# edsonportosilva/OptiCommPy

Measured on AMD Instinct MI355X. Metric: SSFM steps/sec (2-pol, 2^20 samples), higher is better.
Workload: dtype f64

## Files before the change

opticommpy_amd/csrc/engine_fused_impl.h:

```cpp
#pragma once
#include <algorithm>
#include <cstdlib>
#include <vector>

#include "dev_ctx.h"
#include "fused_engine.h"
#include "ssf_internal.h"

namespace ssf {
namespace {

using namespace fused;

#ifdef SSF_PHASE_TIMING
__device__ unsigned long long g_marks[4][4096][8];
#endif

struct DevCtx : DevCtxCore {
#ifdef SSF_PHASE_TIMING
    int kind;
    unsigned long long ts[8] = {0, 0, 0, 0, 0, 0, 0, 0};
    __device__ __forceinline__ void mark(int i) {
        __builtin_amdgcn_sched_barrier(0);
#if SSF_PHASE_TIMING != 2
// ... 244 lines not shown
        if (lg1 == 8 && cols == 8) return pick_col_sg_d<T, 8>(sg);
        if (lg1 == 9 && cols == 8) return pick_col_sg_d<T, 9>(sg);
    } else if constexpr (std::is_same<T, pf2>::value) {
        if (lg1 == 10 && cols == 4) return pick_col_sg_pk<10>(sg);
        if (lg1 == 9 && cols == 8) return pick_col_sg_pk<9>(sg);
    }
    return nullptr;
}
template <typename T> ColFn<T> pick_col(int lg1, int mode) {
    switch (lg1) {
    case 7: return pick_col_mode<T, 7>(mode);
    case 8: return pick_col_mode<T, 8>(mode);
    case 9: return pick_col_mode<T, 9>(mode);
    default: return pick_col_mode<T, 0>(mode);
    }
}

struct HipBackend {
    ssf_plan *pl;
    hipError_t first_err = hipSuccess;
    std::string where;
    hipEvent_t ev0 = nullptr, ev1 = nullptr;

    int row_occ = 2;
    bool col_il = false;
    bool profiling = false;
    struct Stamp { hipEvent_t a, b; int cat; };
    std::vector<Stamp> stamps;
    std::vector<hipEvent_t> pool;
    ssf_kernel_times kt{};
    hipEvent_t get_event() {
        if (!pool.empty()) { hipEvent_t e = pool.back(); pool.pop_back(); return e; }
        hipEvent_t e = nullptr;
        chk(hipEventCreate(&e), "hipEventCreate");
        return e;
    }
    void stamp_begin(int cat) {
        if (!profiling) return;
        Stamp s{get_event(), get_event(), cat};
        chk(hipEventRecord(s.a, pl->stream), "hipEventRecord");
        stamps.push_back(s);
    }
    void stamp_end() {
        if (!profiling) return;
        chk(hipEventRecord(stamps.back().b, pl->stream), "hipEventRecord");
    }
// ... 544 lines not shown
```

opticommpy_amd/csrc/fused_engine.h:

```cpp
#pragma once
#include <algorithm>
#include <cmath>
#include <cstdlib>
#include <cstring>
#include <memory>
#include <string>
#include <type_traits>
#include <vector>

#include "fused_kernels.h"
#include "ssf_derived.h"

namespace ssf {
namespace fused {

#ifndef SSF_EXPERIMENTS
#define SSF_EXPERIMENTS 0
#endif
static inline const char *tune_env(const char *name) {
#if SSF_EXPERIMENTS
    return std::getenv(name);
#else
    (void)name;
    return nullptr;
// ... 111 lines not shown
        }
    }
    return best < 1e300;
}

static inline bool choose_nonpow2_split(int64_t N, int precision, int f1, int fc, bool l1_forced, int *l1, int *N1, int *N2, int *C) {
    *l1 = *N1 = *N2 = *C = 0;
    if (f1 > 0 && choose_mixed2_split(N, precision, N1, N2, C, f1, fc)) return true;
    if (!choose_mixed_split(N, precision, l1, N2)) {
        *l1 = *N2 = 0;
        return choose_mixed2_split(N, precision, N1, N2, C);
    }
    if (*l1 < 7 && !l1_forced) {
        int n1 = 0, n2 = 0, c = 0;
        if (choose_mixed2_split(N, precision, &n1, &n2, &c)) {
            *l1 = 0;
            *N1 = n1;
            *N2 = n2;
            *C = c;
        }
    }
    return true;
}

template <typename T, class Backend> class FusedCore {
  public:
    using C = cx<T>;
    using S = scalar_t<T>;
    static constexpr bool kPacked = sizeof(T) != sizeof(S);
    Backend &be;
    int64_t N;
    int nrows, log2N;
    Split sp;
    int N2mix = 0;
    int mix_rows = 1;
    MixPlan mix_plan{};
    cx<double> *wtab = nullptr;
    int N1mix = 0, mix_cols = 0;
    MixPlan mix_plan1{};
    cx<double> *wtab1 = nullptr;
    int n1() const { return N1mix ? N1mix : 1 << sp.l1; }
    int row_tw_off = 0;
    size_t field_bytes;
    C *G = nullptr, *T0 = nullptr, *T1 = nullptr, *Ehd = nullptr, *noise_d = nullptr;
    S *P = nullptr, *Theta = nullptr;
    bool own_G = true;
    void *cpl_comm = nullptr;
    double *cpl_work = nullptr;
    std::unique_ptr<FusedCore<pf2, Backend>> pk;
    bool use_packed = true;
    bool lim0_bound = true;
    Ctrl *ctrl = nullptr;
    LinOp *linops = nullptr;
    unsigned *gbar = nullptr;
    double *part = nullptr;
    double *tr_hz = nullptr, *tr_lim = nullptr;
    int *tr_it = nullptr;
    long long tr_cap = 0;
    int tr_maxIter = 0;
    std::vector<C *> snaps;
    int row_v = 16;
    int col_v = 16;
    bool underfilled = false;
    int lanes_hint = 1;
    int col_split = 1;
    bool split_ok = true;
    int split_penalty = 0;
    static constexpr int kSplitPenalty = 8;
    int hint_n_it = 0;
    int cur = 0;
    unsigned seq = 0;
    int row_block, row_grid, col_block_mk, col_grid_mk, col_block_1, col_grid_1, npart_max;
    size_t row_lds, col_lds_mk, col_lds_1;
    std::string err;

    std::vector<ssf_stats> ustats;
    int units = 1;
    int npairs() const { return kPacked ? nrows : std::max(nrows / 2, 1); }
    int rows_u() const { return nrows / units; }
    int pairs_u() const { return std::max(npairs() / units, 1); }
    FusedCore(Backend &b, int64_t N_, int nrows_, int precision, void *borrowed_G = nullptr, int units_ = 1)
        : be(b), N(N_), nrows(nrows_), units(units_ > 0 ? units_ : 1) {
        if (borrowed_G) {
            G = (C *)borrowed_G;
            own_G = false;
        }
        log2N = 0;
        while ((1ll << log2N) < N) ++log2N;
        if ((N & (N - 1)) == 0) {
            choose_split(log2N, precision, &sp, kPacked);
        } else {
// ... 16 lines not shown
            *lds = mix2_col_lds(N1mix, mix_cols, npol, (int)sizeof(C));
            return;
        }
        const int tpf = (1 << sp.l1) / col_v, N2 = N2mix ? N2mix : 1 << sp.l2;
        int half = col_v == 8 ? 512 / npol : 256;
        if (const char *e = tune_env("SSF_COL_HALF")) {
            const int h = std::atoi(e);
            if (h >= tpf && h <= 512 && (h & (h - 1)) == 0) half = h;
        }
        while (half / tpf > N2 && half > tpf) half >>= 1;
        auto wgs = [&](int h) { return (long long)groups * (N2 / (h / tpf)); };
        while (!tune_env("SSF_COL_HALF") && half > 64 &&
               ((wgs(half) < 512 && (half / tpf) * sizeof(C) > 128) || (wgs(half) < 256 && (half / tpf) * sizeof(C) > 64)))
            half >>= 1;
        const int Cc = half / tpf;
        *block = half * npol;
        *grid = groups * ((N2 + Cc - 1) / Cc);
        *lds = std::max((size_t)npol * Cc * lds_col_stride(1 << sp.l1, Cc, (int)sizeof(C)) * sizeof(C), (size_t)half * npol * 16 + 1024);
    }

    int init() {
        if (const char *e = tune_env("SSF_LIM0_BOUND")) lim0_bound = std::atoi(e) != 0;
        if (const char *e = tune_env("SSF_COL_SPLIT")) col_split = std::atoi(e);
        underfilled = (double)rows_u() * (double)N <= 1048576.0;
        col_v = underfilled && sp.l1 != 7 ? 8 : 16;
        if (const char *e = tune_env("SSF_COL_V")) col_v = std::atoi(e) == 8 ? 8 : 16;
        if (N2mix || sp.l1 < 6 || sp.l1 > 10) col_v = 16;
        if (N1mix && !mix_make_plan(N1mix, &mix_plan1, 256 / (2 * mix_cols), false)) {
            err = "fused engine: no pass plan for the column length";
            return SSF_ERR_UNSUPPORTED;
        }
        if (const char *e = N1mix ? tune_env("SSF_MIX_PLAN1") : nullptr) {
            int r[kMixMaxPass], n = 0;
            for (const char *q = e; *q && n < kMixMaxPass;) {
                r[n++] = std::atoi(q);
                while (*q && *q != ',') ++q;
                if (*q == ',') ++q;
            }
            MixPlan mp;
            if (mix_plan_from_radices(N1mix, r, n, &mp)) mix_plan1 = mp;
        }
        const int64_t nfft = (int64_t)rows_u() * n1();
        if (N2mix) {
            int tpr = 128;
            if (const char *e = tune_env("SSF_MIX_TPR")) tpr = std::max(64, std::min(1024, std::atoi(e)));
            while (16 * tpr < N2mix) tpr *= 2;
// ... 344 lines not shown

    MkConst mk_const(const ssf_params &p, const Derived &d) const {
        MkConst k{};
        k.Lspan = p.Lspan;
        k.hz_fixed = p.hz;
        k.tol = p.tol;
        k.maxRot = p.maxNlinPhaseRot;
        k.c8g = d.c8g;
        k.sgn = p.direction >= 0 ? 1.0 : -1.0;
        k.lin_a = d.lin_a;
        k.lin_b = d.lin_b;
        k.w2 = (d.w_scale / (double)N) * (d.w_scale / (double)N);
        k.invN = 1.0 / (double)N;
        k.maxIter = p.maxIter;
        k.adaptive = p.nlprMethod ? 1 : 0;
        k.exact_lim0 = (p.maxIter == 1 || !lim0_bound) ? 1 : 0;
        k.log2N = log2N;
        k.trace_cap = tr_cap;
        k.tr_hz = tr_hz;
        k.tr_it = tr_it;
        k.tr_lim = tr_lim;
        return k;
    }
    void launch_mk_row(const MkConst &k) {
        RowArgs<T> a = row_args();
        a.use_ctrl = 1;
        a.cin = ctrl + (size_t)(seq & 1) * units;
        a.cout = ctrl + (size_t)((seq + 1) & 1) * units;
        a.k = k;
        const size_t ps = (size_t)units * (size_t)npart_max;
        a.pmax = part;
        a.pnum = part + ps;
        a.pden = part + 2 * ps;
        a.pnum0 = part + 3 * ps;
        a.pden0 = part + 4 * ps;
        a.npart = col_grid_mk;
        if constexpr (Backend::kCanCouple) {
            if (cpl_comm) {
                if (be.couple(cpl_comm, part, ps, col_grid_mk, cpl_work)) return;
                a.pnum0 = cpl_work;
                a.pden0 = cpl_work + 1;
                a.pnum = cpl_work + 2;
                a.pden = cpl_work + 3;
                a.pmax = cpl_work + 4;
                a.npart = 1;
            }
        }
        be.launch_row(a, row_grid, row_block, row_lds, units);
        ++seq;
// ... 77 lines not shown
                unsigned flags[8] = {0, 0, 0, 0, 0, 0, 0, 0};
                be.d2h(flags, gbar, sizeof(flags));
                if (!be.ok()) return hiperr();
                if (flags[2]) {
                    err = "persistent Manakov kernel: grid barrier timed out (workgroups not co-resident / not on one XCD?)";
                    return SSF_ERR_STATE;
                }
                seq = (seq & ~1u) | (flags[4] & 1u);
                be.d2h(cs.data(), ctrl + (seq & 1), sizeof(Ctrl));
                if (!be.ok()) return hiperr();
                if (cs[0].state != ST_SPAN_DONE || cs[0].pend0) {
                    err = "persistent Manakov kernel: span not finished";
                    return SSF_ERR_STATE;
                }
                persisted = true;
            }
        }
        if (!persisted) {
        launch_mk_col(k, CM_MK);
        int guard = 0;
        long long prev_steps = 0, prev_iters = 0, prev_rare = 0;
        const bool can_split = col_split && split_penalty == 0 && units == 1 && !cpl_comm &&
                               be.can_split_cols(col_args(kPacked ? 1 : 2, CM_MK), col_block_mk);
        bool general_chunk = false;
        int stalls = 0, pos = 0;
        long long idle_pairs = 0;
        for (;;) {
            double steps_rem = 0.0;
            for (const Ctrl &c : cs) {
                double r;
                if (c.state == ST_SPAN_DONE && !c.pend0) r = 0.0;
                else if (c.steps == 0 && c.state == ST_NEED_S) r = p.nlprMethod ? 8.0 : std::ceil(p.Lspan / p.hz);
                else r = std::max(1.0, std::ceil((p.Lspan - c.z) / (c.hz > 0 ? c.hz : p.hz)));
                steps_rem = std::max(steps_rem, r);
            }
            const bool use_split = can_split && split_ok && !general_chunk;
            const int n_pred = std::max(1, std::min(p.maxIter, sr.n_it > 0 ? sr.n_it : (int)std::lround(sr.avg_it)));
            double est = p.nlprMethod ? steps_rem * (1.0 + sr.avg_it) * 0.6
                                      : steps_rem * (1.0 + (use_split ? std::max((double)n_pred, sr.avg_it) : sr.avg_it)) + 3.0;
            int chunk = (int)std::min(512.0, std::max(2.0, std::ceil(est)));
            if (can_split && split_ok && general_chunk) chunk = std::min(chunk, 8);
            else if (use_split && sr.n_it == 0) chunk = std::min(chunk, 4 * (n_pred + 1));
            for (int i = 0; i < chunk; ++i) {
                launch_mk_row(k);
                int sg = SG_ALL;
                if (use_split) {
                    sg = pos == 0 ? (SG_H | SG_RARE) : pos < n_pred ? SG_ADV : SG_FIN;
                    pos = pos >= n_pred ? 0 : pos + 1;
                }
                launch_mk_col(k, CM_MK, sg);
            }
            be.d2h(cs.data(), ctrl + (size_t)(seq & 1) * units, cbytes);
            if (!be.ok()) return hiperr();
            long long steps = 0, iters = 0, rare = 0;
            bool done = true;
            double worst = 0.0;
            for (const Ctrl &c : cs) {
                steps += c.steps;
                iters += c.iterations;
                rare += c.n_rebuilt + c.n_recovered;
                done = done && c.state == ST_SPAN_DONE && !c.pend0;
                if (c.steps > 0) worst = std::max(worst, (double)c.iterations / (double)c.steps);
            }
            if (steps > prev_steps) {
                sr.avg_it = units == 1 ? (double)(iters - prev_iters) / (double)(steps - prev_steps) : worst;
                sr.n_it = cs[0].last_nit;
            }
            if (can_split && split_ok && !done) {
                idle_pairs = steps == prev_steps ? idle_pairs + chunk : 0;
                const bool stuck = idle_pairs >= 2 * (n_pred + 1) + 2;
                if (general_chunk && !stuck) general_chunk = false;
                else if (stuck) {
                    general_chunk = true;
                    if (++stalls >= 2) split_ok = false;
                }
                if (rare - prev_rare > (steps - prev_steps) / 4 + 2) split_ok = false;
                if (!split_ok) split_penalty = kSplitPenalty;
            }
            prev_steps = steps;
            prev_iters = iters;
            prev_rare = rare;
            if (done) break;
            if (++guard > (1 << 22)) {
                err = "fused engine: span did not terminate";
                return SSF_ERR_STATE;
            }
        }
        }
        if (units == 1) {
            cur = cs[0].cur;
        } else {
            const size_t ub = sizeof(C) * (size_t)rows_u() * (size_t)N;
            for (int u = 0; u < units; ++u)
                if (cs[(size_t)u].cur != cur)
// ... 162 lines not shown
```

opticommpy_amd/csrc/fused_kernels.h:

```cpp
#pragma once
#include "fused_core.h"
#include "mixed_fft.h"
#include "ssf_rng.h"

namespace ssf {
namespace fused {

enum {
    ST_NEED_S = 0,
    ST_AFTER_S = 1,
    ST_NEED_H = 2,
    ST_ROW_ITER = 3,
    ST_NEED_I = 4,
    ST_SPAN_DONE = 6,
    ST_REDO0 = 7,
    ST_RECOVER_A = 8,
    ST_RECOVER_ROW = 9,
    ST_RECOVER_B = 10
};

struct LinOp {
    double cth;
    double mag;
    double Cre[9], Cim[9];
};

struct Ctrl {
    int state, it, cur, hz_valid;
    int final_;
    int pend0, pendn;
    int cap0;
    int pcur, redo_;
    int bound0;
    int exact0;
    int t_sparse;
    int dense;
    int gscale;
    int last_nit;
    long long pend0_idx;
    double z, hz;
    long long steps, iterations, nonconv, trace_n;
    long long n_ahead, n_rebuilt;
    long long n_recovered;
    LinOp lin;
};

struct MkConst {
    double Lspan, hz_fixed, tol, maxRot, c8g, sgn, lin_a, lin_b, w2, invN;
    int maxIter, adaptive, log2N;
    int exact_lim0;
    long long trace_cap;
    double *tr_hz;
    int *tr_it;
    double *tr_lim;
};

SSF_HD LinOp make_linop(double hzh, double lin_a, double lin_b, double w2, double invN, int log2N) {
    LinOp l;
    l.cth = lin_b * w2 * hzh;
    l.mag = exp(lin_a * hzh) * invN;
    const double d = (double)(1ll << (log2N - 4));
    for (int m = 0; m < 9; ++m) {
        double s, c;
        cis_rad_d(l.cth * d * d * (double)(m * m), c, s);
        l.Cre[m] = c;
        l.Cim[m] = s;
    }
    return l;
}

SSF_HD double pick_hz(const MkConst &k, double z, double maxphi) {
    if (k.adaptive) {
        const double cand = k.maxRot / maxphi;
        return (k.Lspan - z >= cand) ? cand : k.Lspan - z;
    }
    return (k.Lspan - z < k.hz_fixed) ? k.Lspan - z : k.hz_fixed;
}

SSF_HD cx<double> tw_base(int sign, int j, int lgL) {
    double c, s;
    cis2pi_d(scale_pow2((double)(sign * j), lgL), c, s);
    return mk<double>(c, s);
}
template <int R> SSF_HD void tw_powers(cx<double> w1, cx<double> *p) {
    p[0] = mk<double>(1.0, 0.0);
    p[1] = w1;
    if (R > 2) {
        p[2] = w1 * w1;
        p[3] = p[2] * w1;
    }
    if (R > 4) {
        p[4] = p[2] * p[2];
        p[5] = p[4] * w1;
        p[6] = p[3] * p[3];
        p[7] = p[4] * p[3];
    }
    if (R > 8) {
        p[8] = p[4] * p[4];
#pragma unroll
        for (int s2 = 9; s2 < 16; ++s2) p[s2 < R ? s2 : 0] = p[8] * p[s2 - 8];
// ... 267 lines not shown
    const LinOp *lin;
    const Ctrl *cin;
    Ctrl *cout;
    MkConst k;
    const double *pmax;
    const double *pnum, *pden;
    const double *pnum0, *pden0;
    int npart;
    int N2;
    long long N;
    int mixed;
    MixPlan plan;
    const cx<double> *wtab;
    int rows_per_wg;
    const cx<T> *harr;
    int fwd_only;
    const cx<T> *src;
    int vpt;
    long long u_elems;
    int u_part;
    int prio;
    int tw_off;
    int N1mix;
};
template <typename T> SSF_HD long long row_n1(const RowArgs<T> &a) { return a.N1mix ? (long long)a.N1mix : 1ll << a.log2N1; }

struct Lin16Bases {
    cx<double> A, B1;
    double cth;
};
template <int V = 16> SSF_HD Lin16Bases lin16_bases(double cth, long long k0, int log2N) {
    constexpr int lgV = V == 16 ? 4 : 3;
    const double dk = (double)(1ll << (log2N - lgV));
    const double k0d = (double)k0;
    double s, c;
    Lin16Bases r;
    cis_rad_d(cth * k0d * k0d, c, s);
    r.A = mk<double>(c, s);
    cis_rad_d(2.0 * cth * k0d * dk, c, s);
    r.B1 = mk<double>(c, s);
    r.cth = cth;
    return r;
}
template <int V = 16, typename T> SSF_HD void apply_lin16(const LinOp &lo, const Lin16Bases &lb, cx<T> *v);
template <int V = 16, typename T>
SSF_HD void apply_lin16(const LinOp &lo, long long k0, int log2N, cx<T> *v) {
// ... 40 lines not shown
#if SSF_CTRL_WIDE
    constexpr int kMax = (int)(sizeof(Ctrl) / 8);
    unsigned long long w[kMax];
#pragma unroll
    for (int q = 0; q < kMax; ++q)
        if (q < nwords) w[q] = src[q];
#pragma unroll
    for (int q = 0; q < kMax; ++q)
        if (q < nwords) dst[q] = w[q];
#else
    int i = 0;
    for (; i + 8 <= nwords; i += 8) {
        unsigned long long w[8];
#pragma unroll
        for (int q = 0; q < 8; ++q) w[q] = src[i + q];
#pragma unroll
        for (int q = 0; q < 8; ++q) dst[i + q] = w[q];
    }
    for (; i < nwords; ++i) dst[i] = src[i];
#endif
}

template <typename T, class Ctx>
SSF_HD bool row_ctrl(Ctx &ctx, const RowArgs<T> &a, const double (&part)[2][4], LinOp &lo) {
    LinOp *lsh = (LinOp *)ctx.lds;
    const Ctrl &c = *a.cin;
    const int c_state = c.state, c_it = c.it, c_pend0 = c.pend0, c_pendn = c.pendn, c_cap0 = c.cap0, c_bound0 = c.bound0;
    int n_exact0 = c.exact0;
    const int c_gscale = c.gscale, c_sparse = c.t_sparse;
    int n_state = c_state, n_final = c.final_, n_cap0 = c_cap0, n_hzv = c.hz_valid;
    int add_nonconv = 0, add_ahead = 0;
    const long long c_nonconv = c.nonconv, c_ahead = c.n_ahead;
    double n_hz = c.hz;
    double *red = (double *)(ctx.lds) + 64;
    const bool lead = ctx.bid == 0 && ctx.tid == 0;
    bool act = c_state == ST_AFTER_S || c_state == ST_ROW_ITER || c_state == ST_RECOVER_ROW;
    if (c_pend0 || c_pendn) {
        double s0 = part[0][0] + part[1][0], s1 = part[0][1] + part[1][1];
        double s2 = part[0][2] + part[1][2], s3 = part[0][3] + part[1][3];
        for (int i = ctx.tid + 2 * ctx.nthreads; i < a.npart; i += ctx.nthreads) {
            s0 += a.pnum0[i];
            s1 += a.pden0[i];
            s2 += a.pnum[i];
            s3 += a.pden[i];
        }
        if (c_pend0) block_sum2(ctx, s0, s1, red);
        if (c_pendn) block_sum2(ctx, s2, s3, red);
// ... 37 lines not shown
        ctx.sync();
        if (ctx.tid == 0) {
            const double hz = pick_hz(a.k, c.z, mx);
            lsh[0] = make_linop(hz / 2, a.k.lin_a, a.k.lin_b, a.k.w2, a.k.invN, a.k.log2N);
            ((double *)(lsh + 1))[0] = hz;
        }
        ctx.sync();
        n_hz = ((double *)(lsh + 1))[0];
        lo = lsh[0];
        if (lead) a.cout->lin = lsh[0];
        n_hzv = 1;
        ctx.sync();
    } else if (act && c_state == ST_RECOVER_ROW) {
        ctx.sync();
        if (ctx.tid == 0) lsh[0] = make_linop(-c.hz / 2, a.k.lin_a, a.k.lin_b, a.k.w2, a.k.invN, a.k.log2N);
        ctx.sync();
        lo = lsh[0];
        ctx.sync();
    } else if (act) {
        lo = c.lin;
    }
    if (act && c_state == ST_AFTER_S && c_gscale) lo.mag *= (double)row_n1(a);
    if (act) n_state = c_state == ST_AFTER_S ? ST_NEED_H : c_state == ST_RECOVER_ROW ? ST_RECOVER_B : ST_NEED_I;
    if (lead) {
        ctrl_forward(a.cin, a.cout, (int)((new_lin ? offsetof(Ctrl, lin) : sizeof(Ctrl)) / 8));
        Ctrl *n = a.cout;
        n->state = n_state;
        n->final_ = n_final;
        n->pend0 = 0;
        n->pendn = 0;
        n->cap0 = n_cap0;
        n->bound0 = 0;
        n->exact0 = n_exact0;
        if (n_exact0) n->dense = 1;
        if (act && c_state == ST_AFTER_S) n->gscale = 0;
        n->hz_valid = n_hzv;
        n->hz = n_hz;
        n->nonconv = c_nonconv + add_nonconv;
        n->n_ahead = c_ahead + add_ahead;
    }
    return act;
}

template <typename T> SSF_HD cx<T> lin_at_n(const LinOp &lo, long long k, long long N) {
    const double kk = (double)(k < (N + 1) / 2 ? k : k - N);
    double s, c;
    cis_rad_d(lo.cth * kk * kk, c, s);
    return mk<T>((T)(lo.mag * c), (T)(lo.mag * s));
}

template <typename T, class Ctx> SSF_HD void row_mixed_body(Ctx &ctx, const RowArgs<T> &a, const MixPlan &p) {
    const int L = a.N2, R_ = a.rows_per_wg, T_ = ctx.nthreads / R_;
    const int f = ctx.tid / T_, t = ctx.tid - f * T_;
    cx<T> *x = (cx<T> *)(ctx.lds + 4096) + (size_t)f * L;
    const long long rr = (long long)ctx.bid * R_ + f;
    cx<T> *g = a.G + rr * L;
    const cx<T> *gin = a.src ? a.src + rr * L : g;
    LinOp lo;
// ... 1 lines not shown
#if SSF_EARLY_BASES
    const double cth_pre = a.use_ctrl ? a.cin->lin.cth : (a.lin ? a.lin->cth : 0.0);
#endif
    if (a.use_ctrl) {
#pragma unroll
        for (int u = 0; u < 2; ++u) {
            const int i = ctx.tid + u * ctx.nthreads;
            if (i < a.npart) {
                part[u][0] = a.pnum0[i];
                part[u][1] = a.pden0[i];
                part[u][2] = a.pnum[i];
                part[u][3] = a.pden[i];
            }
        }
        ctx.issue_fence();
    }
    ctx.mark(0);
    const int N1 = (int)row_n1(a);
    const int k1 = a.N1mix ? (int)(rr % N1) : (int)(rr & (N1 - 1));
    MixRowOp op;
    auto ctrl = [&]() {
        if (a.use_ctrl) {
            ctx.issue_fence();
            if (!row_ctrl(ctx, a, part, lo)) return false;
        } else {
            lo = *a.lin;
        }
        const int Rl = p.r[p.npass - 1];
        op.cth = lo.cth;
        op.mag = lo.mag;
        op.D = (double)(a.N / Rl);
        double c, s;
        cis_rad_d(2.0 * lo.cth * op.D * op.D, c, s);
        op.c2 = mk<double>(c, s);
        op.k1 = k1;
        op.N1 = N1;
        op.N = a.N;
        return true;
    };
    if (!mix_dif_op_dit(ctx, p, t, T_, x, a.wtab, op, gin, g, ctrl)) return;
    ctx.mark(4);
    ctx.mark(5);
    ctx.flush(0);
}

#ifndef SSF_WT_ROWS
#define SSF_WT_ROWS 3
#endif
#ifndef SSF_LOAD_ORDER
#define SSF_LOAD_ORDER 1
#endif
#ifndef SSF_EARLY_BASES
#define SSF_EARLY_BASES 0
#endif
#ifndef SSF_SPEC_G
#define SSF_SPEC_G 0
#endif
#ifndef SSF_PAIR_DPP
#define SSF_PAIR_DPP 0
#endif
#ifndef SSF_THETA_F32
#define SSF_THETA_F32 0
#endif
template <typename T> constexpr bool wt_rows() {
    return sizeof(scalar_t<T>) == 8 ? (SSF_WT_ROWS & 1) != 0 : sizeof(T) == 8 ? (SSF_WT_ROWS & 2) != 0 : (SSF_WT_ROWS & 4) != 0;
}
template <int V, typename T, class Ctx>
SSF_HD void row_store(Ctx &ctx, const RowArgs<T> &a, const PassPlan &p, int f, int b, const cx<T> *v) {
    const int fpw = ctx.nthreads / p.tpf;
    cx<T> *base = a.G + (((long long)ctx.bid * fpw) << a.log2N2);
#if defined(__HIP_DEVICE_COMPILE__)
    if constexpr (wt_rows<T>()) {
        const unsigned bytes = (unsigned)(((size_t)fpw << a.log2N2) * sizeof(cx<T>));
        const __amdgpu_buffer_rsrc_t rs = __builtin_amdgcn_make_buffer_rsrc((void *)base, 0, bytes, 0x00020000);
        constexpr int kWT = 0x11;
#pragma unroll
        for (int q = 0; q < V; ++q) {
            const unsigned off = (unsigned)(((f << a.log2N2) + b + p.tpf * q) * (int)sizeof(cx<T>));
            if constexpr (sizeof(cx<T>) == 16) {
                typedef unsigned u4 __attribute__((ext_vector_type(4)));
                u4 w;
                __builtin_memcpy(&w, &v[q], 16);
                __builtin_amdgcn_raw_buffer_store_b128(w, rs, off, 0, kWT);
            } else {
                typedef unsigned u2 __attribute__((ext_vector_type(2)));
                u2 w;
                __builtin_memcpy(&w, &v[q], 8);
                __builtin_amdgcn_raw_buffer_store_b64(w, rs, off, 0, kWT);
            }
        }
        return;
    }
#endif
    cx<T> *g = base + ((long long)f << a.log2N2);
#pragma unroll
    for (int q = 0; q < V; ++q) g[b + p.tpf * q] = v[q];
}

template <typename T, int LG, int V = 16, class Ctx> SSF_HD void row_body(Ctx &ctx, const RowArgs<T> &a) {
    constexpr int lgV = V == 16 ? 4 : 3;
    cx<T> *lds = (cx<T> *)ctx.lds;
    LinOp lo;
    const PassPlan p = make_plan(LG > 0 ? LG : a.log2N2, lgV);
    const int fpw = ctx.nthreads / p.tpf;
    const int f = ctx.tid / p.tpf, b = ctx.tid % p.tpf;
    const long long rr = (long long)ctx.bid * fpw + f;
    cx<T> *g = a.G + (rr << a.log2N2);
    cx<T> v[V];
    ctx.mark(0);
    double part[2][4] = {{0, 0, 0, 0}, {0, 0, 0, 0}};
#if SSF_EARLY_BASES
    const double cth_pre = a.use_ctrl ? a.cin->lin.cth : (a.lin ? a.lin->cth : 0.0);
#endif
    if (a.use_ctrl) {
#pragma unroll
        for (int u = 0; u < 2; ++u) {
            const int i = ctx.tid + u * ctx.nthreads;
            if (i < a.npart) {
                part[u][0] = a.pnum0[i];
                part[u][1] = a.pden0[i];
                part[u][2] = a.pnum[i];
                part[u][3] = a.pden[i];
            }
        }
        ctx.issue_fence();
    }
#if SSF_LOAD_ORDER
    {
        constexpr int ord16[16] = {0, 8, 4, 12, 2, 10, 6, 14, 1, 9, 5, 13, 3, 11, 7, 15};
        constexpr int ord8[8] = {0, 4, 2, 6, 1, 5, 3, 7};
#pragma unroll
        for (int i = 0; i < V; ++i) {
            const int q = V == 16 ? ord16[i] : ord8[i & 7];
            v[q] = g[b + p.tpf * q];
            if ((i & 3) == 3) ctx.issue_fence();
        }
    }
#else
#pragma unroll
    for (int q = 0; q < V; ++q) v[q] = g[b + p.tpf * q];
#endif
    constexpr bool kTab = (SSF_TW_TAB & 1) && sizeof(scalar_t<T>) == 4;
    TwSrc<T> tws;
    if (kTab) {
        tw_entry_t<T> *tab = (tw_entry_t<T> *)(ctx.lds + a.tw_off);
        tw_lds_build<T>(ctx, p, tab);
        tws.lds = tab;
    }
    if (a.use_ctrl) {
        ctx.issue_fence();
        if (!row_ctrl(ctx, a, part, lo)) return;
    } else if (a.lin) {
        lo = *a.lin;
    }
    if (kTab && p.npass == 2) ctx.sync();
    const int N1 = 1 << a.log2N1, log2N = a.log2N1 + a.log2N2;
    const int k1 = (int)(rr & (N1 - 1));
    cx<T> *l = lds + (size_t)f * lds_slots_per_fft(p.L);
    ctx.mark(1);
    if (a.prio) ctx.template setprio<2>();
    const int last = p.npass - 1;
#if SSF_EARLY_BASES
    Lin16Bases lb{};
    const bool lin16 = (a.use_ctrl || a.lin) && p.lg(last) == lgV;
    {
#pragma unroll
        for (int i = 0; i < kTwMaxPass; ++i) {
            if (i < p.npass && p.lgLn(i) > 0 && !(kTab && i == p.npass - 2)) {
                tws.base[i] = tw_base(+1, pass_j(p, i, b), pass_lgLi(p, i));
                tws.have[i] = true;
            }
        }
        if (lin16) lb = lin16_bases<V>(cth_pre, k1 + ((long long)rev_pos(p, reg_pos(p, last, b, 0)) << a.log2N1), log2N);
        ctx.issue_fence();
    }
#endif
    fft_dif<-1, V, kTab>(ctx, p, b, v, l, tws);
    ctx.mark(2);
    if (a.prio) ctx.template setprio<1>();
    if (!a.use_ctrl && !a.lin) {
        if (a.fwd_only) {
#pragma unroll
            for (int idx = 0; idx < V; ++idx) g[reg_pos(p, last, b, idx)] = v[idx];
            return;
        }
        const cx<T> *h = a.harr + ((size_t)k1 << a.log2N2);
#pragma unroll
        for (int idx = 0; idx < V; ++idx) v[idx] = v[idx] * h[reg_pos(p, last, b, idx)];
    } else if (p.lg(last) == lgV) {
#if SSF_EARLY_BASES
        if (lo.cth != lb.cth) lb = lin16_bases<V>(lo.cth, k1 + ((long long)rev_pos(p, reg_pos(p, last, b, 0)) << a.log2N1), log2N);
        apply_lin16<V>(lo, lb, v);
#else
        const long long k0 = k1 + ((long long)rev_pos(p, reg_pos(p, last, b, 0)) << a.log2N1);
        apply_lin16<V>(lo, k0, log2N, v);
#endif
    } else {
#pragma unroll
        for (int idx = 0; idx < V; ++idx) {
            const long long k = k1 + ((long long)rev_pos(p, reg_pos(p, last, b, idx)) << a.log2N1);
            v[idx] = mul_by_d(v[idx], lin_at(lo, k, log2N));
        }
    }
    ctx.mark(3);
    fft_dit<+1, V, kTab>(ctx, p, b, v, l, tws);
    if (a.prio) ctx.template setprio<0>();
    ctx.mark(4);
    row_store<V>(ctx, a, p, f, b, v);
    ctx.mark(5);
    ctx.flush(0);
}

enum {
    CM_NLSE_FIRST = 0,
    CM_NLSE_STEP = 1,
    CM_NLSE_LAST = 2,
    CM_MK = 3,
    CM_PLAIN_FWD = 5,
    CM_PLAIN_INV = 6
};

template <typename T> struct ColArgs {
    cx<T> *G;
    cx<T> *T0, *T1;
    cx<T> *Ehd;
    scalar_t<T> *P;
    scalar_t<T> *Theta;
    int log2N1, log2N2, npol, mode;
    int ngroups;
    scalar_t<T> g_hz;
    const Ctrl *cin;
// ... 319 lines not shown
        const double s = sin_half_angle((double)ang - (double)prev);
        theta_st(g, a.Theta, g.pbase + t, ang);
        shC[(size_t)own_idx(g, j) * g.half + g.t] = cis_t<T>(ang);
        shD[(size_t)own_idx(g, j) * g.half + g.t] = (T)(4.0 * s * s);
    }
    ctx.mark(7);
#pragma unroll
    for (int idx = H; idx < V; ++idx) v[idx] = g.ld(a.Ehd, g.rowbase + g.time_off(idx));
    ctx.sync();
#pragma unroll
    for (int idx = 0; idx < V; ++idx) {
        const cx<T> e = v[idx];
        const double w = (double)norm2(e);
        num += w * (double)shD[(size_t)idx * g.half + g.t];
        den += w;
        v[idx] = e * shC[(size_t)idx * g.half + g.t];
    }
    ctx.sync();
}

struct MkColStage {
    bool do_inv = false, do_fwd = false, final_ = false, more = false, exact0 = true;
    bool sparse = false;
    int op = -1;
    struct { int state, it, cur, pcur; double z, hz; } c{};
};
template <int V> SSF_HD bool lim0_bound_sample(int idx, int b) { return idx == 0 && (V == 16 || !(b & 1)); }
enum { SG_H = 1, SG_ADV = 2, SG_FIN = 4, SG_RARE = 8, SG_ALL = 15 };
SSF_HD int stage_group(int op, bool final_) { return op == 1 ? SG_H : op == 2 ? (final_ ? SG_FIN : SG_ADV) : SG_RARE; }
template <class Ctx, class Args> SSF_HD void mk_col_stage(Ctx &ctx, const Args &a, MkColStage &st, int sg_mask = SG_ALL) {
    bool &do_inv = st.do_inv, &do_fwd = st.do_fwd, &final_ = st.final_, &more = st.more, &exact0 = st.exact0;
    int &op = st.op;
    auto &c = st.c;
    c.state = a.cin->state;
    c.it = a.cin->it;
    c.cur = a.cin->cur;
    c.pcur = a.cin->pcur;
    c.z = a.cin->z;
    c.hz = a.cin->hz;
    final_ = a.cin->final_ != 0;
    exact0 = a.k.exact_lim0 || a.cin->exact0 != 0;
    const int c_exact0 = a.cin->exact0, c_redo = a.cin->redo_;
    const long long c_trace_n = a.cin->trace_n, c_steps = a.cin->steps, c_iters = a.cin->iterations;
    const long long c_rebuilt = a.cin->n_rebuilt, c_recovered = a.cin->n_recovered;
    if (c.state == ST_NEED_S) {
        op = 0;
        do_fwd = true;
    } else if (c.state == ST_NEED_H) {
        op = 1;
        do_inv = do_fwd = true;
    } else if (c.state == ST_NEED_I) {
        op = 2;
        do_inv = true;
        more = c.z + c.hz < a.k.Lspan;
        do_fwd = final_ ? false : true;
        st.sparse = final_ && more && !a.k.exact_lim0 && !a.cin->dense &&
                    (a.k.adaptive || pick_hz(a.k, c.z + c.hz, 0.0) == c.hz);
    } else if (c.state == ST_REDO0) {
        op = 3;
        do_fwd = true;
    } else if (c.state == ST_RECOVER_A) {
        op = 4;
        do_fwd = true;
    } else if (c.state == ST_RECOVER_B) {
        op = 5;
        do_inv = do_fwd = true;
    }
    if (op >= 0 && !(stage_group(op, final_) & sg_mask)) {
        op = -1;
        do_inv = do_fwd = false;
    }
    if (ctx.bid == 0 && ctx.tid == 0) {
        ctrl_forward(a.cin, a.cout, (int)(sizeof(Ctrl) / 8));
        Ctrl *n = a.cout;
        if (op == 0) {
            n->state = ST_AFTER_S;
            n->gscale = 0;
            n->t_sparse = n->dense = 0;
            n->hz_valid = 0;
        } else if (op == 1) {
            n->state = ST_ROW_ITER;
            n->it = 0;
            n->final_ = a.k.maxIter == 1;
            n->pend0 = n->pendn = 0;
        } else if (op == 4) {
            n->state = ST_RECOVER_ROW;
        } else if (op == 3 || op == 5) {
            if (op == 5) n->t_sparse = 0;
            n->state = ST_ROW_ITER;
            n->it = 0;
            n->final_ = c_exact0 ? 0 : 1;
            n->redo_ = c_exact0 ? 0 : 1;
            n->pend0 = n->pendn = 0;
            n->n_rebuilt = c_rebuilt + 1;
            if (op == 5) n->n_recovered = c_recovered + 1;
        } else if (op == 2 && !final_) {
            n->state = ST_ROW_ITER;
            n->it = c.it + 1;
            n->pendn = 1;
            if (c.it == 0) {
                n->pend0 = 1;
                n->pend0_idx = c_trace_n;
                n->bound0 = exact0 ? 0 : 1;
                n->exact0 = 0;
            }
        } else if (op == 2) {
            const long long tn = c_trace_n;
// ... 5 lines not shown
            n->steps = c_steps + 1;
            n->iterations = c_iters + c.it + 1;
            n->last_nit = c.it + 1;
            n->z = c.z + c.hz;
            n->cur = c.cur ^ 1;
            n->it = 0;
            n->final_ = 0;
            if (c.it == 0) {
                n->pend0 = 1;
                n->pend0_idx = tn;
                n->cap0 = c_redo ? 0 : 1;
                n->bound0 = exact0 ? 0 : 1;
                n->exact0 = 0;
            }
            n->redo_ = 0;
            n->t_sparse = st.sparse ? 1 : 0;
            n->dense = 0;
            if (more) {
                n->gscale = 1;
                n->state = ST_AFTER_S;
                n->pcur = c.pcur ^ 1;
                if (a.k.adaptive) n->hz_valid = 0;
                else {
                    const double hz = pick_hz(a.k, c.z + c.hz, 0.0);
                    if (hz != c.hz) n->hz_valid = 0;
                    n->hz = hz;
                }
            } else n->state = ST_SPAN_DONE;
        }
    }
}

#define G_DPP(g) (std::remove_reference<decltype(g)>::type::kDppT && (g).dpp)
template <typename T, int LG, int MODE, bool RAGGED, int V = 16, int CI = 0, int SG = SG_ALL, class Ctx>
SSF_HD void col_body(Ctx &ctx, const ColArgs<T> &a) {
    constexpr int H = V / 2;
    constexpr int kCI = CI > 0 ? CI : 1;
    constexpr bool kMk = MODE == CM_MK;
    constexpr bool kgH = (SG & SG_H) != 0, kgADV = (SG & SG_ADV) != 0, kgFIN = (SG & SG_FIN) != 0, kgRARE = (SG & SG_RARE) != 0;
    constexpr bool kFwd = !kMk || kgH || kgADV || kgRARE;
    bool do_inv = false, do_fwd = false;
    int op = -1;
    bool final_ = false, more = false, exact0 = true, sparse = false;
    struct { int state, it, cur, pcur; double z, hz; } c{};
    double *red = (double *)ctx.lds;
    ctx.mark(0);
    ColGeom<T, LG, Ctx, RAGGED, V> g(ctx, a);
    cx<T> v[V];
#if SSF_SPEC_G
    if (kMk) {
#pragma unroll
        for (int q = 0; q < V; ++q) {
            v[q] = g.ld(a.G, g.rowbase + g.freq_off(q));
            if ((q & 3) == 3) ctx.issue_fence();
        }
    }
#endif
    if (kMk) {
        MkColStage st;
        mk_col_stage(ctx, a, st, SG);
        do_inv = st.do_inv;
        do_fwd = kFwd && st.do_fwd;
        final_ = kgFIN && (!kgADV || st.final_);
        more = st.more;
        exact0 = st.exact0;
        sparse = st.sparse;
        op = st.op;
        c.state = st.c.state;
        c.it = st.c.it;
        c.cur = st.c.cur;
        c.pcur = st.c.pcur;
        c.z = st.c.z;
        c.hz = st.c.hz;
        if (op < 0) return;
    } else {
        do_inv = MODE == CM_NLSE_STEP || MODE == CM_NLSE_LAST || MODE == CM_PLAIN_INV;
        do_fwd = MODE == CM_NLSE_STEP || MODE == CM_NLSE_FIRST || MODE == CM_PLAIN_FWD;
    }

    const PassPlan &p = g.p;
    cx<T> *lds = CI > 0 ? (cx<T> *)ctx.lds + (size_t)g.pol * CI * lds_slots_per_fft(p.L) + g.c
                        : (cx<T> *)ctx.lds + (size_t)(g.pol * g.C + g.c) * lds_col_stride(p.L, g.C, (int)sizeof(cx<T>));

    cx<T> *Tcur = a.T0, *Tnew = a.T1;
    T *Pcur = a.P, *Palt = a.P;
    if (kMk) {
        Tcur = c.cur ? a.T1 : a.T0;
        Tnew = c.cur ? a.T0 : a.T1;
        const long long psz = g.N * a.ngroups;
        Pcur = a.P + (c.pcur ? psz : 0);
        Palt = a.P + (c.pcur ? 0 : psz);
    }

    TwSrc<T> tws;
    GTw gtw;
    cx<T> e_pre{};
    if (do_inv) {
        if (!(kMk && SSF_SPEC_G)) {
#pragma unroll
            for (int q = 0; q < V; ++q) {
                v[q] = g.ld(a.G, g.rowbase + g.freq_off(q));
#if SSF_LOAD_ORDER
                if ((q & 3) == 3) ctx.issue_fence();
#endif
            }
        }
        if (kMk && (kgADV || kgFIN) && op == 2 && c.it == 0 && !exact0 && lim0_bound_sample<V>(0, g.b)) e_pre = g.ld(Tcur, g.rowbase + g.time_off(0));
        ctx.mark(1);
        if (a.prio) ctx.template setprio<3>();
        global_twiddle<+1, RAGGED>(g, a.log2N1 + a.log2N2, v, gtw);
        fft_dif<+1, V, false, kCI>(ctx, p, g.b, v, lds, tws);
        ctx.mark(2);
        if (a.prio) ctx.template setprio<2>();
    } else if (kMk && !kgRARE) {
    } else if (!(kMk && op == 3)) {
        const cx<T> *src = kMk && op == 4 ? a.Ehd : Tcur;
#pragma unroll
        for (int idx = 0; idx < V; ++idx) v[idx] = g.ld(src, g.rowbase + g.time_off(idx));
    }

    if (MODE == CM_NLSE_STEP) {
#pragma unroll
        for (int idx = 0; idx < V; ++idx) v[idx] = v[idx] * cis_t<T>(a.g_hz * norm2(v[idx]));
    } else if (MODE == CM_NLSE_LAST || MODE == CM_PLAIN_INV) {
// ... 776 lines not shown
```

Before: 6321.

## Pair row kernel passes to compute next step's linear half-step ahead

When the step has converged on a fixed step size, the row kernel now runs a second FFT-linear-IFFT trip inside the same launch. It writes the next step's half-step linear result into the alternate T buffer and sets a half_ahead flag in the control block. The host loop then skips the following row launch, and the column kernel reads G from that alternate buffer. The aim is to save a full row pass, with its launch and global memory round trip, on fixed-step NLSE iterations, at the cost of more control-state complexity and a looped row kernel body that may raise register pressure.

```diff
diff --git a/opticommpy_amd/csrc/engine_fused_impl.h b/opticommpy_amd/csrc/engine_fused_impl.h
--- a/opticommpy_amd/csrc/engine_fused_impl.h
+++ b/opticommpy_amd/csrc/engine_fused_impl.h
@@ -290,6 +290,7 @@
     std::string where;
     hipEvent_t ev0 = nullptr, ev1 = nullptr;
 
+    static constexpr bool kCanPairRows = true;
     int row_occ = 2;
     bool col_il = false;
     bool profiling = false;
diff --git a/opticommpy_amd/csrc/fused_engine.h b/opticommpy_amd/csrc/fused_engine.h
--- a/opticommpy_amd/csrc/fused_engine.h
+++ b/opticommpy_amd/csrc/fused_engine.h
@@ -157,6 +157,9 @@
     }
     return true;
 }
+
+template <class B, class = void> struct backend_pairs_rows : std::false_type {};
+template <class B> struct backend_pairs_rows<B, std::void_t<decltype(B::kCanPairRows)>> : std::integral_constant<bool, B::kCanPairRows> {};
 
 template <typename T, class Backend> class FusedCore {
   public:
@@ -202,6 +205,7 @@
     bool split_ok = true;
     int split_penalty = 0;
     static constexpr int kSplitPenalty = 8;
+    int pair_rows = backend_pairs_rows<Backend>::value ? 1 : 0;
     int hint_n_it = 0;
     int cur = 0;
     unsigned seq = 0;
@@ -264,6 +268,7 @@
     int init() {
         if (const char *e = tune_env("SSF_LIM0_BOUND")) lim0_bound = std::atoi(e) != 0;
         if (const char *e = tune_env("SSF_COL_SPLIT")) col_split = std::atoi(e);
+        if (const char *e = tune_env("SSF_PAIR")) pair_rows = std::max(0, std::min(2, std::atoi(e)));
         underfilled = (double)rows_u() * (double)N <= 1048576.0;
         col_v = underfilled && sp.l1 != 7 ? 8 : 16;
         if (const char *e = tune_env("SSF_COL_V")) col_v = std::atoi(e) == 8 ? 8 : 16;
@@ -654,9 +659,12 @@
         k.tr_lim = tr_lim;
         return k;
     }
-    void launch_mk_row(const MkConst &k) {
+    void launch_mk_row(const MkConst &k, bool pair = false) {
         RowArgs<T> a = row_args();
         a.use_ctrl = 1;
+        a.pair = pair ? 1 : 0;
+        a.T0 = T0;
+        a.T1 = T1;
         a.cin = ctrl + (size_t)(seq & 1) * units;
         a.cout = ctrl + (size_t)((seq + 1) & 1) * units;
         a.k = k;
@@ -780,7 +788,10 @@
         long long prev_steps = 0, prev_iters = 0, prev_rare = 0;
         const bool can_split = col_split && split_penalty == 0 && units == 1 && !cpl_comm &&
                                be.can_split_cols(col_args(kPacked ? 1 : 2, CM_MK), col_block_mk);
-        bool general_chunk = false;
+        const bool can_pair = can_split && pair_rows > 0 && !p.nlprMethod && !kPacked && std::is_same<T, double>::value &&
+                              row_v == 16 && col_v == 16 && !N2mix && !N1mix;
+        bool general_chunk = false, skip_row = false;
+        double zp = 0.0, hzp = 0.0;
         int stalls = 0, pos = 0;
         long long idle_pairs = 0;
         for (;;) {
@@ -799,13 +810,28 @@
             int chunk = (int)std::min(512.0, std::max(2.0, std::ceil(est)));
             if (can_split && split_ok && general_chunk) chunk = std::min(chunk, 8);
             else if (use_split && sr.n_it == 0) chunk = std::min(chunk, 4 * (n_pred + 1));
+            const bool pairing = can_pair && use_split;
+            if (can_pair && pair_rows == 2) chunk = std::min(chunk, n_pred + 1);
+            if (pairing) {
+                const Ctrl &c0 = cs[0];
+                zp = c0.z;
+                hzp = c0.hz_valid ? c0.hz : pick_hz(k, c0.z, 0.0);
+                if (pos == 0) skip_row = c0.state == ST_NEED_H && c0.g_alt;
+            }
             for (int i = 0; i < chunk; ++i) {
-                launch_mk_row(k);
                 int sg = SG_ALL;
+                bool row = true;
                 if (use_split) {
                     sg = pos == 0 ? (SG_H | SG_RARE) : pos < n_pred ? SG_ADV : SG_FIN;
+                    if (pairing && pos == 0 && skip_row) row = false;
+                    if (pairing && sg == SG_FIN) {
+                        skip_row = sr.n_it >= 2 && zp + hzp < k.Lspan && next_fixed_hz(k, zp, hzp) == hzp;
+                        zp += hzp;
+                        hzp = pick_hz(k, zp, 0.0);
+                    }
                     pos = pos >= n_pred ? 0 : pos + 1;
                 }
+                if (row) launch_mk_row(k, pairing);
                 launch_mk_col(k, CM_MK, sg);
             }
             be.d2h(cs.data(), ctrl + (size_t)(seq & 1) * units, cbytes);
@@ -828,6 +854,7 @@
                 idle_pairs = steps == prev_steps ? idle_pairs + chunk : 0;
                 const bool stuck = idle_pairs >= 2 * (n_pred + 1) + 2;
                 if (general_chunk && !stuck) general_chunk = false;
+                else if (can_pair && pair_rows == 2 && !stuck && pos == 0) general_chunk = true;
                 else if (stuck) {
                     general_chunk = true;
                     if (++stalls >= 2) split_ok = false;
diff --git a/opticommpy_amd/csrc/fused_kernels.h b/opticommpy_amd/csrc/fused_kernels.h
--- a/opticommpy_amd/csrc/fused_kernels.h
+++ b/opticommpy_amd/csrc/fused_kernels.h
@@ -37,6 +37,8 @@
     int dense;
     int gscale;
     int last_nit;
+    int half_ahead;
+    int g_alt;
     long long pend0_idx;
     double z, hz;
     long long steps, iterations, nonconv, trace_n;
@@ -76,6 +78,7 @@
     }
     return (k.Lspan - z < k.hz_fixed) ? k.Lspan - z : k.hz_fixed;
 }
+SSF_HD double next_fixed_hz(const MkConst &k, double z, double hz) { return pick_hz(k, z + hz, 0.0); }
 
 SSF_HD cx<double> tw_base(int sign, int j, int lgL) {
     double c, s;
@@ -389,6 +392,8 @@
     int prio;
     int tw_off;
     int N1mix;
+    int pair;
+    cx<T> *T0, *T1;
 };
 template <typename T> SSF_HD long long row_n1(const RowArgs<T> &a) { return a.N1mix ? (long long)a.N1mix : 1ll << a.log2N1; }
 
@@ -475,7 +480,8 @@
 }
 
 template <typename T, class Ctx>
-SSF_HD bool row_ctrl(Ctx &ctx, const RowArgs<T> &a, const double (&part)[2][4], LinOp &lo) {
+SSF_HD bool row_ctrl(Ctx &ctx, const RowArgs<T> &a, const double (&part)[2][4], LinOp &lo, int &pair_cur) {
+    pair_cur = -1;
     LinOp *lsh = (LinOp *)ctx.lds;
     const Ctrl &c = *a.cin;
     const int c_state = c.state, c_it = c.it, c_pend0 = c.pend0, c_pendn = c.pendn, c_cap0 = c.cap0, c_bound0 = c.bound0;
@@ -559,6 +565,12 @@
     }
     if (act && c_state == ST_AFTER_S && c_gscale) lo.mag *= (double)row_n1(a);
     if (act) n_state = c_state == ST_AFTER_S ? ST_NEED_H : c_state == ST_RECOVER_ROW ? ST_RECOVER_B : ST_NEED_I;
+    bool paired = false;
+    if (a.pair && act && c_state == ST_ROW_ITER && n_final && c_it >= 1 && !c.redo_ && !a.k.adaptive) {
+        const double z = c.z, hz = c.hz;
+        paired = z + hz < a.k.Lspan && next_fixed_hz(a.k, z, hz) == hz;
+        if (paired) pair_cur = c.cur;
+    }
     if (lead) {
         ctrl_forward(a.cin, a.cout, (int)((new_lin ? offsetof(Ctrl, lin) : sizeof(Ctrl)) / 8));
         Ctrl *n = a.cout;
@@ -571,6 +583,7 @@
         n->exact0 = n_exact0;
         if (n_exact0) n->dense = 1;
         if (act && c_state == ST_AFTER_S) n->gscale = 0;
+        if (paired) n->half_ahead = 1;
         n->hz_valid = n_hzv;
         n->hz = n_hz;
         n->nonconv = c_nonconv + add_nonconv;
@@ -618,7 +631,8 @@
     auto ctrl = [&]() {
         if (a.use_ctrl) {
             ctx.issue_fence();
-            if (!row_ctrl(ctx, a, part, lo)) return false;
+            int pair_cur;
+            if (!row_ctrl(ctx, a, part, lo, pair_cur)) return false;
         } else {
             lo = *a.lin;
         }
@@ -658,13 +672,22 @@
 #ifndef SSF_THETA_F32
 #define SSF_THETA_F32 0
 #endif
+#ifndef SSF_PAIR_KEEP
+#define SSF_PAIR_KEEP 0
+#endif
+SSF_HD int opaque_int(int x) {
+#if defined(__HIP_DEVICE_COMPILE__)
+    asm volatile("" : "+v"(x));
+#endif
+    return x;
+}
 template <typename T> constexpr bool wt_rows() {
     return sizeof(scalar_t<T>) == 8 ? (SSF_WT_ROWS & 1) != 0 : sizeof(T) == 8 ? (SSF_WT_ROWS & 2) != 0 : (SSF_WT_ROWS & 4) != 0;
 }
 template <int V, typename T, class Ctx>
-SSF_HD void row_store(Ctx &ctx, const RowArgs<T> &a, const PassPlan &p, int f, int b, const cx<T> *v) {
+SSF_HD void row_store(Ctx &ctx, const RowArgs<T> &a, cx<T> *dst, const PassPlan &p, int f, int b, const cx<T> *v) {
     const int fpw = ctx.nthreads / p.tpf;
-    cx<T> *base = a.G + (((long long)ctx.bid * fpw) << a.log2N2);
+    cx<T> *base = dst + (((long long)ctx.bid * fpw) << a.log2N2);
 #if defined(__HIP_DEVICE_COMPILE__)
     if constexpr (wt_rows<T>()) {
         const unsigned bytes = (unsigned)(((size_t)fpw << a.log2N2) * sizeof(cx<T>));
@@ -699,7 +722,7 @@
     LinOp lo;
     const PassPlan p = make_plan(LG > 0 ? LG : a.log2N2, lgV);
     const int fpw = ctx.nthreads / p.tpf;
-    const int f = ctx.tid / p.tpf, b = ctx.tid % p.tpf;
+    const int f0 = ctx.tid / p.tpf, b0 = ctx.tid % p.tpf, f = f0, b = b0;
     const long long rr = (long long)ctx.bid * fpw + f;
     cx<T> *g = a.G + (rr << a.log2N2);
     cx<T> v[V];
@@ -743,21 +766,22 @@
         tw_lds_build<T>(ctx, p, tab);
         tws.lds = tab;
     }
+    constexpr bool kPairs = V == 16 && sizeof(T) == 8 && sizeof(scalar_t<T>) == 8;
+    int pair_cur = -1;
     if (a.use_ctrl) {
         ctx.issue_fence();
-        if (!row_ctrl(ctx, a, part, lo)) return;
+        if (!row_ctrl(ctx, a, part, lo, pair_cur)) return;
     } else if (a.lin) {
         lo = *a.lin;
     }
     if (kTab && p.npass == 2) ctx.sync();
     const int N1 = 1 << a.log2N1, log2N = a.log2N1 + a.log2N2;
-    const int k1 = (int)(rr & (N1 - 1));
-    cx<T> *l = lds + (size_t)f * lds_slots_per_fft(p.L);
+    [[maybe_unused]] const int k1 = (int)(rr & (N1 - 1));
     ctx.mark(1);
     if (a.prio) ctx.template setprio<2>();
     const int last = p.npass - 1;
+    Lin16Bases lb{};
 #if SSF_EARLY_BASES
-    Lin16Bases lb{};
     const bool lin16 = (a.use_ctrl || a.lin) && p.lg(last) == lgV;
     {
 #pragma unroll
@@ -771,38 +795,60 @@
         ctx.issue_fence();
     }
 #endif
-    fft_dif<-1, V, kTab>(ctx, p, b, v, l, tws);
-    ctx.mark(2);
-    if (a.prio) ctx.template setprio<1>();
-    if (!a.use_ctrl && !a.lin) {
-        if (a.fwd_only) {
-#pragma unroll
-            for (int idx = 0; idx < V; ++idx) g[reg_pos(p, last, b, idx)] = v[idx];
-            return;
-        }
-        const cx<T> *h = a.harr + ((size_t)k1 << a.log2N2);
-#pragma unroll
-        for (int idx = 0; idx < V; ++idx) v[idx] = v[idx] * h[reg_pos(p, last, b, idx)];
-    } else if (p.lg(last) == lgV) {
+    cx<T> *dst = a.G;
+#if SSF_PAIR_COPY
+#pragma unroll
+#else
+#pragma unroll 1
+#endif
+    for (int trip = 0; trip < 2; ++trip) {
+        const int b = opaque_int(b0), f = opaque_int(f0);
+        const int k1 = (int)(((long long)ctx.bid * fpw + f) & (N1 - 1));
+        cx<T> *l = lds + (size_t)f * lds_slots_per_fft(p.L);
+        fft_dif<-1, V, kTab>(ctx, p, b, v, l, tws);
+        ctx.mark(2);
+        if (a.prio) ctx.template setprio<1>();
+        if (!a.use_ctrl && !a.lin) {
+            if (a.fwd_only) {
+#pragma unroll
+                for (int idx = 0; idx < V; ++idx) g[reg_pos(p, last, b, idx)] = v[idx];
+                return;
+            }
+            const cx<T> *h = a.harr + ((size_t)k1 << a.log2N2);
+#pragma unroll
+            for (int idx = 0; idx < V; ++idx) v[idx] = v[idx] * h[reg_pos(p, last, b, idx)];
+        } else if (p.lg(last) == lgV) {
 #if SSF_EARLY_BASES
-        if (lo.cth != lb.cth) lb = lin16_bases<V>(lo.cth, k1 + ((long long)rev_pos(p, reg_pos(p, last, b, 0)) << a.log2N1), log2N);
-        apply_lin16<V>(lo, lb, v);
+            if (lo.cth != lb.cth) lb = lin16_bases<V>(lo.cth, k1 + ((long long)rev_pos(p, reg_pos(p, last, b, 0)) << a.log2N1), log2N);
 #else
-        const long long k0 = k1 + ((long long)rev_pos(p, reg_pos(p, last, b, 0)) << a.log2N1);
-        apply_lin16<V>(lo, k0, log2N, v);
-#endif
-    } else {
-#pragma unroll
-        for (int idx = 0; idx < V; ++idx) {
-            const long long k = k1 + ((long long)rev_pos(p, reg_pos(p, last, b, idx)) << a.log2N1);
-            v[idx] = mul_by_d(v[idx], lin_at(lo, k, log2N));
-        }
-    }
-    ctx.mark(3);
-    fft_dit<+1, V, kTab>(ctx, p, b, v, l, tws);
-    if (a.prio) ctx.template setprio<0>();
-    ctx.mark(4);
-    row_store<V>(ctx, a, p, f, b, v);
+            if (trip == 0 || !(SSF_PAIR_KEEP & 1)) lb = lin16_bases<V>(lo.cth, k1 + ((long long)rev_pos(p, reg_pos(p, last, b, 0)) << a.log2N1), log2N);
+#endif
+            apply_lin16<V>(lo, lb, v);
+        } else {
+#pragma unroll
+            for (int idx = 0; idx < V; ++idx) {
+                const long long k = k1 + ((long long)rev_pos(p, reg_pos(p, last, b, idx)) << a.log2N1);
+                v[idx] = mul_by_d(v[idx], lin_at(lo, k, log2N));
+            }
+        }
+        ctx.mark(3);
+        fft_dit<+1, V, kTab>(ctx, p, b, v, l, tws);
+        if (a.prio) ctx.template setprio<0>();
+        ctx.mark(4);
+        row_store<V>(ctx, a, dst, p, f, b, v);
+        if (!kPairs || pair_cur < 0 || trip) break;
+        if (SSF_PAIR_KEEP & 4) lo.mag *= (double)row_n1(a);
+        else {
+            lo = a.cin->lin;
+            lo.mag *= (double)row_n1(a);
+        }
+        if (!(SSF_PAIR_KEEP & 2)) {
+#pragma unroll
+            for (int i = 0; i < kTwMaxPass; ++i) tws.have[i] = false;
+        }
+        dst = pair_cur ? a.T1 : a.T0;
+        if (a.prio) ctx.template setprio<2>();
+    }
     ctx.mark(5);
     ctx.flush(0);
 }
@@ -1168,6 +1214,7 @@
 struct MkColStage {
     bool do_inv = false, do_fwd = false, final_ = false, more = false, exact0 = true;
     bool sparse = false;
+    bool g_alt = false;
     int op = -1;
     struct { int state, it, cur, pcur; double z, hz; } c{};
 };
@@ -1186,7 +1233,8 @@
     c.hz = a.cin->hz;
     final_ = a.cin->final_ != 0;
     exact0 = a.k.exact_lim0 || a.cin->exact0 != 0;
-    const int c_exact0 = a.cin->exact0, c_redo = a.cin->redo_;
+    const int c_exact0 = a.cin->exact0, c_redo = a.cin->redo_, c_half = a.cin->half_ahead;
+    st.g_alt = a.cin->g_alt != 0;
     const long long c_trace_n = a.cin->trace_n, c_steps = a.cin->steps, c_iters = a.cin->iterations;
     const long long c_rebuilt = a.cin->n_rebuilt, c_recovered = a.cin->n_recovered;
     if (c.state == ST_NEED_S) {
@@ -1201,7 +1249,7 @@
         more = c.z + c.hz < a.k.Lspan;
         do_fwd = final_ ? false : true;
         st.sparse = final_ && more && !a.k.exact_lim0 && !a.cin->dense &&
-                    (a.k.adaptive || pick_hz(a.k, c.z + c.hz, 0.0) == c.hz);
+                    (a.k.adaptive || next_fixed_hz(a.k, c.z, c.hz) == c.hz);
     } else if (c.state == ST_REDO0) {
         op = 3;
         do_fwd = true;
@@ -1229,6 +1277,7 @@
             n->it = 0;
             n->final_ = a.k.maxIter == 1;
             n->pend0 = n->pendn = 0;
+            n->g_alt = 0;
         } else if (op == 4) {
             n->state = ST_RECOVER_ROW;
         } else if (op == 3 || op == 5) {
@@ -1280,9 +1329,15 @@
                 n->pcur = c.pcur ^ 1;
                 if (a.k.adaptive) n->hz_valid = 0;
                 else {
-                    const double hz = pick_hz(a.k, c.z + c.hz, 0.0);
+                    const double hz = next_fixed_hz(a.k, c.z, c.hz);
                     if (hz != c.hz) n->hz_valid = 0;
                     n->hz = hz;
+                }
+                if (c_half) {
+                    n->state = ST_NEED_H;
+                    n->gscale = 0;
+                    n->half_ahead = 0;
+                    n->g_alt = 1;
                 }
             } else n->state = ST_SPAN_DONE;
         }
@@ -1300,6 +1355,7 @@
     bool do_inv = false, do_fwd = false;
     int op = -1;
     bool final_ = false, more = false, exact0 = true, sparse = false;
+    bool g_alt = false;
     struct { int state, it, cur, pcur; double z, hz; } c{};
     double *red = (double *)ctx.lds;
     ctx.mark(0);
@@ -1331,6 +1387,7 @@
         c.z = st.c.z;
         c.hz = st.c.hz;
         if (op < 0) return;
+        g_alt = kgH && op == 1 && st.g_alt;
     } else {
         do_inv = MODE == CM_NLSE_STEP || MODE == CM_NLSE_LAST || MODE == CM_PLAIN_INV;
         do_fwd = MODE == CM_NLSE_STEP || MODE == CM_NLSE_FIRST || MODE == CM_PLAIN_FWD;
@@ -1354,10 +1411,11 @@
     GTw gtw;
     cx<T> e_pre{};
     if (do_inv) {
-        if (!(kMk && SSF_SPEC_G)) {
+        if (!(kMk && SSF_SPEC_G) || g_alt) {
+            const cx<T> *Gsrc = g_alt ? Tnew : a.G;
 #pragma unroll
             for (int q = 0; q < V; ++q) {
-                v[q] = g.ld(a.G, g.rowbase + g.freq_off(q));
+                v[q] = g.ld(Gsrc, g.rowbase + g.freq_off(q));
 #if SSF_LOAD_ORDER
                 if ((q & 3) == 3) ctx.issue_fence();
 #endif
```

New measurement: 5817. 8.0% lower.
